# deepika090/HL-HGAT

Hardware: AMD Instinct MI355X
Metric: graphs/sec HL-HGAT fwd+bwd, ZINC-12k simplex graphs, 1/2/4/8 MI355X (higher is better)
Workload: dtype fp32; 1 GPU; BASELINE configs[1]: ZINC-12k-scale, HL_HGCNN_zinc_dense_int3_pyr channels=[2,2,2] filters=[64,64,64] K=3 mlp=[256,256] keig=15; step = copy of the device-resident batch into the step's static buffers + fwd + L1 + bwd (+ grad all-reduce) + Adam; the batch tables (Laplacian / incidence CSRs, degrees, segment offsets) are built by the data loader at collate time, outside the step (see loader); graphs_per_gpu=1000, global_batch=1000, parallelism=dp1

## Files before the change

hl-hgat_amd/csrc/bn.hip:

```cpp
#include "gemm_core.h"

#include <atomic>
#include <cstdlib>

using namespace hlhgat;

namespace {

constexpr int kThreads = 256;
constexpr int kMaxParts = 512;
constexpr int kFlatMax = 256;
constexpr int kGroup = 16;
constexpr int kMaxGroups = kMaxParts / kGroup;
constexpr int kMaxTiles = 1024;
constexpr int kGridBase = kMaxTiles * (1 + kMaxGroups);
constexpr int kCounters = kGridBase + 2 * kMaxTiles;
constexpr int kMaxSlots = 4096;
constexpr int APPLY_RPT = 2;
constexpr int kMaxRpt = 32;

struct BnLayout {
  int v;
  int tpr;
  int rp;
// ... 92 lines not shown
}

struct StatsArgs {
  const int32_t* nvalid;
  const float* x;
  int64_t ldx;
  const float* y;
  int64_t ldy;
  const float* dy;
  int64_t lddy;
  int64_t n;
  int C;
  int tpr, rp, tiles, parts;
  int64_t rows_per_part;
  double* part;
  double* gpart;
  unsigned* count;
  const float* weight;
  const float* bias;
  float* running_mean;
  float* running_var;
  int64_t* nbt;
  float momentum, eps;
  float* save_mean;
  float* save_invstd;
  float* coef;
  float* dweight;
  float* dbias;
  float* out;
  int64_t ldo;
  int relu;
  unsigned wait_us;
  unsigned* err;
  unsigned long long* slots;
  double* sums_out;
  int flat_max;
};

typedef __attribute__((address_space(1))) unsigned long long gu64_t;
__device__ __forceinline__ void st_wt(double* p, double v) {
  __hip_atomic_store((gu64_t*)p, (unsigned long long)__double_as_longlong(v), __ATOMIC_RELAXED,
                     __HIP_MEMORY_SCOPE_AGENT);
}
__device__ __forceinline__ double ld_wt(const double* p) {
  return __longlong_as_double(
      (long long)__hip_atomic_load((gu64_t*)p, __ATOMIC_RELAXED, __HIP_MEMORY_SCOPE_AGENT));
}

__device__ unsigned g_bn_wait_timeouts = 0;
__device__ unsigned g_bn_log_n = 0;
__device__ hlhgat_bn_giveup_t g_bn_log[HLHGAT_BN_LOG_MAX];

constexpr uint64_t kTicksPerUs = 100;
enum : unsigned { kKidBnGrid = 1, kKidProjBn = 2 };

__device__ __forceinline__ void report_state_error(unsigned* err) {
  if (err) __hip_atomic_store(err, (unsigned)HLHGAT_DEVERR_BN_STATE, __ATOMIC_RELAXED,
                              __HIP_MEMORY_SCOPE_SYSTEM);
}

__device__ __forceinline__ bool arrive_last(unsigned* counter, unsigned total, unsigned* err) {
  __shared__ unsigned s_last;
  asm volatile("s_waitcnt vmcnt(0)" ::: "memory");
  __syncthreads();
  if (threadIdx.x == 0) {
    unsigned prev = __hip_atomic_fetch_add(counter, 1u, __ATOMIC_RELAXED,
                                           __HIP_MEMORY_SCOPE_AGENT);
    s_last = (prev == total - 1) ? 1u : 0u;
    if (prev >= total) report_state_error(err);
    if (s_last)
      __hip_atomic_store(counter, 0u, __ATOMIC_RELAXED, __HIP_MEMORY_SCOPE_AGENT);
  }
  __syncthreads();
  return s_last != 0u;
}

typedef __attribute__((address_space(1))) unsigned long long gu64c_t;

__device__ __forceinline__ unsigned long long slot_mark(unsigned gen0) {
  return ((unsigned long long)gen0 << 2) | 1ull;
}

__device__ __forceinline__ bool poll_gen(unsigned long long* word, unsigned gen0,
                                         unsigned wait_us) {
  const uint64_t t0 = __builtin_amdgcn_s_memrealtime();
  const uint64_t lim = (uint64_t)wait_us * kTicksPerUs;
  for (;;) {
    const unsigned long long w =
        __hip_atomic_load((gu64c_t*)word, __ATOMIC_RELAXED, __HIP_MEMORY_SCOPE_AGENT);
    if ((unsigned)(w >> 32) != gen0) return true;
    if (__builtin_amdgcn_s_memrealtime() - t0 >= lim) return false;
    __builtin_amdgcn_s_sleep(2);
  }
}

__device__ __forceinline__ bool give_up(unsigned long long* word, unsigned long long* slot,
                                        unsigned gen0, unsigned kid, const unsigned* arr,
                                        bool arr_low64, unsigned total, unsigned wait_us) {
  const unsigned long long mark = slot_mark(gen0);
  __hip_atomic_store((gu64c_t*)slot, mark, __ATOMIC_SEQ_CST, __HIP_MEMORY_SCOPE_AGENT);
  const unsigned long long w =
      __hip_atomic_load((gu64c_t*)word, __ATOMIC_SEQ_CST, __HIP_MEMORY_SCOPE_AGENT);
  bool mine = false;
  if ((unsigned)(w >> 32) != gen0) {
    unsigned long long exp = mark;
    mine = __hip_atomic_compare_exchange_strong((gu64c_t*)slot, &exp, mark + 1ull,
                                                __ATOMIC_SEQ_CST, __ATOMIC_SEQ_CST,
// ... 460 lines not shown
        if (a.y) yv[u] = vload<V>(a.y + rr * a.ldy + c);
      }
#pragma unroll
      for (int u = 0; u < 4; ++u) acc(xv[u], gv[u], yv[u]);
    }
    for (; r < r_hi; r += a.rp) {
      vt xv = vload<V>(a.x + r * a.ldx + c);
      vt gv = vload<V>(a.dy + r * a.lddy + c);
      vt yv = gv;
      if (a.y) yv = vload<V>(a.y + r * a.ldy + c);
      acc(xv, gv, yv);
    }
  }
  write_partials<V, kThreads>(s0, s1, a, c0, blk);
  __shared__ double sum0[kThreads], sum1[kThreads];
  const int tile_c = a.tpr * V;
  if (!last_reduce<kThreads>(a, c0, tile_c, sum0, sum1, blk)) return;
  if (a.sums_out) {
    write_sums(a, c0, tile_c, sum0, sum1, n_eff, blk);
    for (int t = threadIdx.x; t < tile_c; t += kThreads) {
      const int cc = c0 + t;
      if (cc >= a.C) continue;
      if (a.dweight) a.dweight[cc] = (float)(sum1[t] * (double)a.save_invstd[cc]);
      if (a.dbias) a.dbias[cc] = (float)sum0[t];
    }
    return;
  }
  for (int t = threadIdx.x; t < tile_c; t += kThreads) {
    const int cc = c0 + t;
    if (cc >= a.C) continue;
    float A, B, Cc;
    bwd_coefs(a.save_invstd[cc], a.weight ? a.weight[cc] : 1.f, sum0[t], sum1[t], n_eff, A, B,
              Cc);
    if (a.dweight) a.dweight[cc] = (float)(sum1[t] * (double)a.save_invstd[cc]);
    if (a.dbias) a.dbias[cc] = (float)sum0[t];
    a.coef[cc] = A;
    a.coef[a.C + cc] = B;
    a.coef[2 * a.C + cc] = Cc;
  }
}

template <int V>
__global__ __launch_bounds__(kThreads) void k_bn_bwd_reduce(StatsArgs a) {
  k_bn_bwd_reduce_body<V>(a, blk_hw());
}

void launch_bwd_reduce(bool vec, dim3 grid, hipStream_t st, ProfScope* prof, const StatsArgs& s) {
  if (vec)
    launch(k_bn_bwd_reduce<4>, grid, dim3(kThreads), 0, st, prof, s);
  else
    launch(k_bn_bwd_reduce<1>, grid, dim3(kThreads), 0, st, prof, s);
}

template <int V>
__device__ __forceinline__ void k_bn_bwd_apply_body(const BwdApplyArgs& a, Blk blk) {
  using vt = typename VecT<V>::type;
  const int cl = threadIdx.x % a.tpr;
  const int rg = threadIdx.x / a.tpr;
  const int c = blk.y * a.tpr * V + cl * V;
  if (c >= a.C) return;
  float A[V], B[V], Cc[V], mu[V];
#pragma unroll
  for (int v = 0; v < V; ++v) {
    A[v] = a.coef[c + v];
    B[v] = a.coef[a.C + c + v];
    Cc[v] = a.coef[2 * a.C + c + v];
    mu[v] = a.mean[c + v];
  }
  const int64_t n_eff = eff_rows(a.n, a.nvalid);
  const int64_t r0 = (int64_t)blk.x * a.rp * APPLY_RPT + rg;
  vt xv[APPLY_RPT], gv[APPLY_RPT], yv[APPLY_RPT];
#pragma unroll
  for (int u = 0; u < APPLY_RPT; ++u) {
    const int64_t r = r0 + u * a.rp;
    if (r < n_eff) {
      xv[u] = vload<V>(a.x + r * a.ldx + c);
      gv[u] = vload<V>(a.dy + r * a.lddy + c);
      if (a.y) yv[u] = vload<V>(a.y + r * a.ldy + c);
    }
  }
#pragma unroll
  for (int u = 0; u < APPLY_RPT; ++u) {
    const int64_t r = r0 + u * a.rp;
    if (r >= a.n) break;
    vt o;
#pragma unroll
    for (int v = 0; v < V; ++v) {
      float g = vget(gv[u], v);
      if (a.y && !(vget(yv[u], v) > 0.f)) g = 0.f;
      vget(o, v) = r >= n_eff ? 0.f : A[v] * g + (B[v] * (vget(xv[u], v) - mu[v]) + Cc[v]);
    }
    vstore<V>(a.dx + r * a.lddx + c, o);
  }
}

template <int V>
__global__ __launch_bounds__(kThreads) void k_bn_bwd_apply(BwdApplyArgs a) {
  k_bn_bwd_apply_body<V>(a, blk_hw());
}

struct SyncArgs {
  const int32_t* nvalid;
  const float* x;
  int64_t ldx;
  const float* y;
  int64_t ldy;
  const float* dy;
  int64_t lddy;
  float* out;
  int64_t ldo;
  int64_t n;
  int C;
  int tpr, rp;
  const double* gathered;
  int world;
  const float* weight;
  const float* bias;
  float* running_mean;
  float* running_var;
  int64_t* nbt;
  float momentum, eps;
  float* save_mean;
  float* save_invstd;
  int relu;
};

__device__ __forceinline__ void sync_totals(const SyncArgs& a, int cc, double& s0, double& s1,
                                            double& cnt) {
  s0 = s1 = cnt = 0.0;
  const int64_t stride = 2 * (int64_t)a.C + 1;
  for (int r = 0; r < a.world; ++r) {
    const double* g = a.gathered + r * stride;
    s0 += g[cc];
    s1 += g[a.C + cc];
    cnt += g[2 * a.C];
  }
}

template <int V>
__global__ __launch_bounds__(kThreads) void k_bn_sync_apply(SyncArgs a) {
  using vt = typename VecT<V>::type;
  const int cl = threadIdx.x % a.tpr;
  const int rg = threadIdx.x / a.tpr;
// ... 364 lines not shown
    }
  }
  __syncthreads();
#pragma unroll
  for (int tn = 0; tn < kPbTN; ++tn) {
    const int cl = tn * 16 + i, cc = n_base + cl;
    const float sc = (s.weight ? s.weight[cc] : 1.f) * ss[cl];
    const float mu = sm[cl];
    const float sh = s.bias ? s.bias[cc] : 0.f;
#pragma unroll
    for (int r = 0; r < 4; ++r) {
      const float z = (acc[tn][r] - mu) * sc + sh;
      acc[tn][r] = m_base + 4 * q + r >= n_eff ? 0.f : ((s.relu && z < 0.f) ? 0.f : z);
    }
  }
  const bool vy = (s.ldo % 4) == 0 && (reinterpret_cast<uintptr_t>(s.out) & 15) == 0;
  store_tile_rows<kPbTN>(acc, scratch, m_base, g.M, s.out + n_base, s.ldo, kPbTN * 16, nullptr,
                         0, vy);
  pb_stamp<STAMPS>(a, 5, pb_now());
  if (!top) return;
  __shared__ unsigned char taken[kMaxParts];
  if (!take_left<kThreads>(tile_slots, parts, s_gen0, taken)) return;
  __builtin_amdgcn_fence(__ATOMIC_ACQUIRE, "agent");
  const int c4 = threadIdx.x & 15, rr = threadIdx.x >> 4;
  float sc[4], mu[4], sh[4];
#pragma unroll
  for (int v = 0; v < 4; ++v) {
    const int cl = 4 * c4 + v, cc = n_base + cl;
    sc[v] = (s.weight ? s.weight[cc] : 1.f) * ss[cl];
    mu[v] = sm[cl];
    sh[v] = s.bias ? s.bias[cc] : 0.f;
  }
  for (int p = 0; p < parts; ++p) {
    if (!taken[p]) continue;
    for (int64_t r = (int64_t)p * 64 + rr; r < (int64_t)p * 64 + 64 && r < g.M; r += 16) {
      float4 xv;
      const float* xp = g.C + r * g.ldc + n_base + 4 * c4;
      if (vx) xv = *reinterpret_cast<const float4*>(xp);
      else xv = make_float4(xp[0], xp[1], xp[2], xp[3]);
      const float4 o = bn_row_out<4>(xv, mu, sc, sh, r >= n_eff, s.relu);
      float* yp = s.out + r * s.ldo + n_base + 4 * c4;
      if (vy) {
        *reinterpret_cast<float4*>(yp) = o;
      } else {
        yp[0] = o.x;
        yp[1] = o.y;
        yp[2] = o.z;
        yp[3] = o.w;
      }
    }
  }
}

bool& proj_bn_fused_flag() {
  static bool v = true;
  return v;
}

bool& proj_bn_split_flag() {
  static bool v = false;
  return v;
}

bool bn_vec_ok(int64_t C, std::initializer_list<int64_t> lds,
               std::initializer_list<const void*> ptrs) {
  if (C % 4) return false;
  for (int64_t ld : lds)
    if (ld % 4) return false;
  for (const void* p : ptrs)
    if (p && !aligned16(p)) return false;
  return true;
}

unsigned apply_grid_x(int64_t n, int rp) {
  int64_t g = ceil_div(n, (int64_t)rp * APPLY_RPT);
  if (g < 1) g = 1;
  return (unsigned)g;
}

StatsArgs stats_args(const BnLayout& L, const BnWs& w, const float* x, int64_t ldx, int64_t n,
                     const int32_t* n_valid, int64_t C) {
  StatsArgs s{};
  s.nvalid = n_valid;
  s.x = x;
  s.ldx = ldx;
  s.n = n;
  s.C = (int)C;
  s.tpr = L.tpr;
  s.rp = L.rp;
  s.tiles = L.tiles;
  s.parts = L.parts;
  s.rows_per_part = L.rows_per_part;
  s.part = w.part;
  s.gpart = w.gpart;
  s.count = w.count;
  s.slots = w.slots;
  s.err = hlhgat::device_error_word();
  s.flat_max = kFlatMax;
  return s;
}

unsigned g_wait_us = 1000;

int64_t capacity_of(const void* kernel) {
  static auto* cache = new std::vector<std::pair<const void*, int64_t>>();
  for (const auto& kv : *cache)
    if (kv.first == kernel) return kv.second;
  int dev = 0, cus = 0, occ = 0;
  int64_t c = 0;
  static const int share = [] {
    const char* e = std::getenv("HLHGAT_BN_COLOCATE");
    const int v = e ? std::atoi(e) : 2;
    return v >= 1 && v <= 16 ? v : 2;
  }();
  if (hipGetDevice(&dev) == hipSuccess &&
      hipDeviceGetAttribute(&cus, hipDeviceAttributeMultiprocessorCount, dev) == hipSuccess &&
      hipOccupancyMaxActiveBlocksPerMultiprocessor(&occ, kernel, kThreads, 0) == hipSuccess)
    c = (int64_t)occ * cus / share;
  cache->push_back({kernel, c});
  return c;
}

int rpt_bucket(const BnLayout& L) {
  const int64_t need = ceil_div(L.rows_per_part, (int64_t)L.rp);
  if (need > kMaxRpt) return 0;
  for (int r : {2, 4, 8, 16, 32})
    if (need <= r) return r;
  return 0;
}


using GridFn = void (*)(StatsArgs);

GridFn fwd_grid_fn(bool vec, int rpt) {
  switch (rpt * 2 + (vec ? 1 : 0)) {
    case 4: return k_bn_fwd_grid<1, 2>;
    case 5: return k_bn_fwd_grid<4, 2>;
    case 8: return k_bn_fwd_grid<1, 4>;
    case 9: return k_bn_fwd_grid<4, 4>;
    case 16: return k_bn_fwd_grid<1, 8>;
    case 17: return k_bn_fwd_grid<4, 8>;
    case 32: return k_bn_fwd_grid<1, 16>;
    case 33: return k_bn_fwd_grid<4, 16>;
    case 64: return k_bn_fwd_grid<1, 32>;
    case 65: return k_bn_fwd_grid<4, 32>;
    default: return nullptr;
  }
}

GridFn pick_grid(const BnLayout& L, bool vec) {
  if (!bn_one_launch() || L.parts > kFlatMax) return nullptr;
  const int64_t grid = (int64_t)L.parts * L.tiles;
  const int rpt = rpt_bucket(L);
  GridFn f = rpt ? fwd_grid_fn(vec, rpt) : nullptr;
  const int64_t cap = f ? capacity_of(reinterpret_cast<const void*>(f)) : 0;
  if (!f || grid > 256 || grid > cap) return nullptr;
  return f;
}


}


extern "C" int64_t hlhgat_bn_workspace_bytes(int64_t n, int64_t C) {
  if (n < 0 || C <= 0) return 0;
  return (int64_t)bn_ws_bytes(n, C);
}

extern "C" int hlhgat_bn_stats_train(const float* x, int64_t ldx, int64_t n,
                                     const int32_t* n_valid, int64_t C, float* running_mean,
                                     float* running_var, int64_t* num_batches_tracked,
                                     float momentum, float eps, float* save_mean,
                                     float* save_invstd, void* workspace,
                                     int64_t workspace_bytes, void* stream) {
  HLH_CHECK_ARG(n >= 1 && C >= 1 && C < (1 << 20) && ldx >= C,
                "bn_stats_train: bad sizes n=%lld C=%lld", (long long)n, (long long)C);
  HLH_CHECK_ARG(x && save_mean && save_invstd, "bn_stats_train: NULL pointer");
  HLH_CHECK_ARG((running_mean == nullptr) == (running_var == nullptr),
                "bn_stats_train: running_mean/var must both be given or both NULL");
  HLH_CHECK_ARG(workspace && workspace_bytes >= (int64_t)bn_ws_bytes(n, C),
                "bn_stats_train: workspace too small");
  const bool vec = bn_vec_ok(C, {ldx}, {x});
  BnLayout L = bn_layout(n, C, vec);
  HLH_CHECK_ARG(L.tiles <= kMaxTiles, "bn_stats_train: C too large");
  StatsArgs s = stats_args(L, carve(workspace, n, C), x, ldx, n, n_valid, C);
  s.running_mean = running_mean;
  s.running_var = running_var;
  s.nbt = num_batches_tracked;
  s.momentum = momentum;
  s.eps = eps;
  s.save_mean = save_mean;
  s.save_invstd = save_invstd;
  hipStream_t st = as_stream(stream);
  dim3 g1(L.parts, L.tiles);
  if (vec)
    launch(k_bn_stats<4>, dim3(g1), dim3(kThreads), 0, st, nullptr, s);
  else
    launch(k_bn_stats<1>, dim3(g1), dim3(kThreads), 0, st, nullptr, s);
  HLH_CHECK_LAUNCH();
  return HLHGAT_OK;
}

extern "C" int hlhgat_bn_apply(const float* x, int64_t ldx, int64_t n, const int32_t* n_valid,
                               int64_t C, const float* weight, const float* bias,
                               const float* save_mean, const float* save_invstd, int relu,
                               float* y, int64_t ldy, void* stream) {
  HLH_CHECK_ARG(n >= 1 && C >= 1 && C < (1 << 20) && ldx >= C && ldy >= C,
                "bn_apply: bad sizes n=%lld C=%lld", (long long)n, (long long)C);
  HLH_CHECK_ARG(x && y && save_mean && save_invstd, "bn_apply: NULL pointer");
  const bool vec = bn_vec_ok(C, {ldx, ldy}, {x, y});
  BnLayout L = bn_layout(n, C, vec);
  HLH_CHECK_ARG(L.tiles <= kMaxTiles, "bn_apply: C too large");
// ... 211 lines not shown
      launch(k_bn_apply<1>, g2, dim3(kThreads), 0, st, nullptr, p);
    HLH_CHECK_LAUNCH();
  }
  return HLHGAT_OK;
}

extern "C" int hlhgat_set_proj_bn_split(int on) {
  proj_bn_split_flag() = on != 0;
  return HLHGAT_OK;
}

extern "C" int hlhgat_set_proj_bn_fused(int on) {
  proj_bn_fused_flag() = on != 0;
  return HLHGAT_OK;
}

extern "C" int hlhgat_proj_bn_fused_capacity(int64_t* out) {
  HLH_CHECK_ARG(out, "proj_bn_fused_capacity: NULL pointer");
  *out = capacity_of(reinterpret_cast<const void*>(k_proj_bn_fwd<false>));
  return HLHGAT_OK;
}

extern "C" int hlhgat_bn_bwd_train(const float* x, int64_t ldx, const float* y,
                                   int64_t ldy, const float* dy, int64_t lddy,
                                   int64_t n, const int32_t* n_valid, int64_t C,
                                   const float* weight,
                                   const float* save_mean, const float* save_invstd,
                                   float* dx, int64_t lddx, float* dweight,
                                   float* dbias, void* workspace,
                                   int64_t workspace_bytes, void* stream) {
  HLH_CHECK_ARG(n >= 1 && C >= 1 && ldx >= C && lddy >= C && lddx >= C && (!y || ldy >= C),
                "bn_bwd_train: bad sizes");
  HLH_CHECK_ARG(x && dy && dx && save_mean && save_invstd, "bn_bwd_train: NULL pointer");
  HLH_CHECK_ARG(workspace && workspace_bytes >= (int64_t)bn_ws_bytes(n, C),
                "bn_bwd_train: workspace too small");
  const bool vec = bn_vec_ok(C, {ldx, lddy, lddx, y ? ldy : 4}, {x, y, dy, dx});
  BnLayout L = bn_layout(n, C, vec, bn_bwd_min_parts());
  HLH_CHECK_ARG(L.tiles <= kMaxTiles, "bn_bwd_train: C too large");
  BnWs w = carve(workspace, n, C);
  StatsArgs s = stats_args(L, w, x, ldx, n, n_valid, C);
  s.flat_max = bn_bwd_flat_max();
  s.y = y;
  s.ldy = ldy;
  s.dy = dy;
  s.lddy = lddy;
  s.weight = weight;
  s.save_mean = const_cast<float*>(save_mean);
  s.save_invstd = const_cast<float*>(save_invstd);
  s.coef = w.coef;
  s.dweight = dweight;
  s.dbias = dbias;
  hipStream_t st = as_stream(stream);
  dim3 g1(L.parts, L.tiles);
  {
    ProfScope prof(HLHGAT_PROF_BN_BWD, st, (y ? 12.0 : 8.0) * (double)n * C, 0.0);
    if (vec)
      launch_bwd_reduce(true, g1, st, &prof, s);
    else
      launch_bwd_reduce(false, g1, st, &prof, s);
  }
  HLH_CHECK_LAUNCH();
  BwdApplyArgs p{n_valid, x, ldx, y, ldy, dy, lddy, dx, lddx, n, (int)C, w.coef, save_mean,
                 L.tpr, L.rp};
  dim3 g2(apply_grid_x(n, L.rp), L.tiles);
  if (vec)
    launch(k_bn_bwd_apply<4>, dim3(g2), dim3(kThreads), 0, st, nullptr, p);
  else
    launch(k_bn_bwd_apply<1>, dim3(g2), dim3(kThreads), 0, st, nullptr, p);
  HLH_CHECK_LAUNCH();
  return HLHGAT_OK;
}

extern "C" int hlhgat_bn_bwd_reduce(const float* x, int64_t ldx, const float* y, int64_t ldy,
                                    const float* dy, int64_t lddy, int64_t n,
                                    const int32_t* n_valid, int64_t C, const float* weight,
                                    const float* save_mean, const float* save_invstd,
                                    float* coef, float* dweight, float* dbias, void* workspace,
                                    int64_t workspace_bytes, void* stream) {
  HLH_CHECK_ARG(n >= 1 && C >= 1 && ldx >= C && lddy >= C && (!y || ldy >= C),
                "bn_bwd_reduce: bad sizes");
  HLH_CHECK_ARG(x && dy && coef && save_mean && save_invstd, "bn_bwd_reduce: NULL pointer");
  HLH_CHECK_ARG(workspace && workspace_bytes >= (int64_t)bn_ws_bytes(n, C),
                "bn_bwd_reduce: workspace too small");
  const bool vec = bn_vec_ok(C, {ldx, lddy, y ? ldy : 4}, {x, y, dy});
  BnLayout L = bn_layout(n, C, vec, bn_bwd_min_parts());
  HLH_CHECK_ARG(L.tiles <= kMaxTiles, "bn_bwd_reduce: C too large");
  BnWs w = carve(workspace, n, C);
  StatsArgs s = stats_args(L, w, x, ldx, n, n_valid, C);
  s.flat_max = bn_bwd_flat_max();
  s.y = y;
  s.ldy = ldy;
  s.dy = dy;
  s.lddy = lddy;
  s.weight = weight;
  s.save_mean = const_cast<float*>(save_mean);
  s.save_invstd = const_cast<float*>(save_invstd);
  s.coef = coef;
  s.dweight = dweight;
  s.dbias = dbias;
  hipStream_t st = as_stream(stream);
  ProfScope prof(HLHGAT_PROF_BN_BWD, st, (y ? 12.0 : 8.0) * (double)n * C, 0.0);
  if (vec)
    launch_bwd_reduce(true, dim3(L.parts, L.tiles), st, &prof, s);
  else
    launch_bwd_reduce(false, dim3(L.parts, L.tiles), st, &prof, s);
  HLH_CHECK_LAUNCH();
// ... 105 lines not shown
    launch_bwd_reduce(false, dim3(g1), as_stream(stream), nullptr, s);
  HLH_CHECK_LAUNCH();
  return HLHGAT_OK;
}

extern "C" int hlhgat_bn_sync_bwd_apply(const float* x, int64_t ldx, const float* y,
                                        int64_t ldy, const float* dy, int64_t lddy, int64_t n,
                                        const int32_t* n_valid, int64_t C, const float* weight,
                                        const float* save_mean, const float* save_invstd,
                                        const double* gathered, int world, float* dx,
                                        int64_t lddx, void* stream) {
  HLH_CHECK_ARG(n >= 1 && C >= 1 && ldx >= C && lddy >= C && lddx >= C && (!y || ldy >= C) &&
                    world >= 1,
                "bn_sync_bwd_apply: bad sizes");
  HLH_CHECK_ARG(x && dy && dx && gathered && save_mean && save_invstd,
                "bn_sync_bwd_apply: NULL pointer");
  const bool vec = bn_vec_ok(C, {ldx, lddy, lddx, y ? ldy : 4}, {x, y, dy, dx});
  const BnLayout L = bn_layout(n, C, vec);
  SyncArgs a{};
  a.nvalid = n_valid;
  a.x = x;
  a.ldx = ldx;
  a.y = y;
  a.ldy = ldy;
  a.dy = dy;
  a.lddy = lddy;
  a.out = dx;
  a.ldo = lddx;
  a.n = n;
  a.C = (int)C;
  a.tpr = L.tpr;
  a.rp = L.rp;
  a.gathered = gathered;
  a.world = world;
  a.weight = weight;
  a.save_mean = const_cast<float*>(save_mean);
  a.save_invstd = const_cast<float*>(save_invstd);
  dim3 g2(apply_grid_x(n, L.rp), L.tiles);
  if (vec)
    launch(k_bn_sync_bwd_apply<4>, dim3(g2), dim3(kThreads), 0, as_stream(stream), nullptr, a);
  else
    launch(k_bn_sync_bwd_apply<1>, dim3(g2), dim3(kThreads), 0, as_stream(stream), nullptr, a);
  HLH_CHECK_LAUNCH();
  return HLHGAT_OK;
}

extern "C" int hlhgat_set_bn_one_launch(int on) {
  bn_one_launch_flag() = on != 0;
  return HLHGAT_OK;
}

extern "C" int hlhgat_get_bn_one_launch(void) { return bn_one_launch_flag() ? 1 : 0; }

extern "C" int hlhgat_set_bn_wait_us(unsigned wait_us) {
  g_wait_us = wait_us;
  return HLHGAT_OK;
}

extern "C" int hlhgat_bn_wait_timeouts(unsigned* out) {
  HLH_CHECK_ARG(out, "bn_wait_timeouts: NULL pointer");
  HLH_CHECK_HIP(hipMemcpyFromSymbol(out, HIP_SYMBOL(g_bn_wait_timeouts), sizeof(unsigned)));
  return HLHGAT_OK;
}

extern "C" int hlhgat_bn_giveup_log(hlhgat_bn_giveup_t* out, int max, int* logged) {
  HLH_CHECK_ARG(logged && (max <= 0 || out), "bn_giveup_log: NULL pointer");
  unsigned n = 0;
  HLH_CHECK_HIP(hipMemcpyFromSymbol(&n, HIP_SYMBOL(g_bn_log_n), sizeof(unsigned)));
  *logged = (int)n;
  int k = (int)n < HLHGAT_BN_LOG_MAX ? (int)n : HLHGAT_BN_LOG_MAX;
  if (k > max) k = max;
  if (k > 0)
    HLH_CHECK_HIP(hipMemcpyFromSymbol(out, HIP_SYMBOL(g_bn_log), sizeof(hlhgat_bn_giveup_t) * k));
  return HLHGAT_OK;
}

extern "C" int hlhgat_bn_giveup_reset(void) {
  const unsigned z = 0;
  HLH_CHECK_HIP(hipDeviceSynchronize());
  HLH_CHECK_HIP(hipMemcpyToSymbol(HIP_SYMBOL(g_bn_log_n), &z, sizeof(unsigned)));
  HLH_CHECK_HIP(hipMemcpyToSymbol(HIP_SYMBOL(g_bn_wait_timeouts), &z, sizeof(unsigned)));
  return HLHGAT_OK;
}
```

hl-hgat_amd/csrc/runtime.hip:

```cpp
#include "common.h"

#include <cstring>
#include <mutex>
#include <vector>

namespace hlhgat {

static thread_local std::string g_last_error;

void set_error(const char* fmt, ...) {
  char buf[1024];
  va_list ap;
  va_start(ap, fmt);
  vsnprintf(buf, sizeof(buf), fmt, ap);
  va_end(ap);
  g_last_error = buf;
}

namespace {
constexpr int kPoolSize = 1 << 14;
struct ProfClass {
  bool enabled = false;
  std::vector<hipEvent_t> start, stop;
  std::vector<double> bytes, flops;
  int used = 0;
  int64_t dropped = 0;
};
std::mutex g_prof_mu;
ProfClass g_prof[HLHGAT_PROF_NCLASS];
}

ProfScope::ProfScope(int kernel_class, hipStream_t s, double b, double f)
    : cls(kernel_class), bytes(b), flops(f) {
  (void)s;
  if (kernel_class < 0 || kernel_class >= HLHGAT_PROF_NCLASS) return;
  std::lock_guard<std::mutex> lk(g_prof_mu);
  ProfClass& pc = g_prof[kernel_class];
  if (!pc.enabled) return;
  if (pc.used >= (int)pc.start.size()) {
    pc.dropped++;
    return;
  }
  slot = pc.used++;
  pc.bytes[slot] = b;
  pc.flops[slot] = f;
  start_ev = pc.start[slot];
  stop_ev = pc.stop[slot];
}

namespace {
std::mutex g_err_mu;
unsigned* g_err_word = nullptr;
}

unsigned* device_error_word() {
  std::lock_guard<std::mutex> lk(g_err_mu);
  if (!g_err_word) {
    void* p = nullptr;
    hipError_t e = hipHostMalloc(&p, 64, hipHostMallocPortable | hipHostMallocMapped |
                                             hipHostMallocCoherent);
    if (e != hipSuccess) {
      set_error("hipHostMalloc(device error word) failed: %s", hipGetErrorString(e));
      return nullptr;
    }
    *static_cast<volatile unsigned*>(p) = 0u;
    g_err_word = static_cast<unsigned*>(p);
  }
  return g_err_word;
}

}

using namespace hlhgat;

extern "C" int hlhgat_version(void) { return 103; }

extern "C" int hlhgat_device_errors(unsigned* out) {
  HLH_CHECK_ARG(out, "device_errors: NULL pointer");
  unsigned* w = device_error_word();
  HLH_CHECK_ARG(w, "device_errors: %s", hlhgat_last_error());
  *out = *static_cast<volatile unsigned*>(w);
  return HLHGAT_OK;
}

extern "C" int hlhgat_clear_device_errors(void) {
  unsigned* w = device_error_word();
  HLH_CHECK_ARG(w, "clear_device_errors: %s", hlhgat_last_error());
  *static_cast<volatile unsigned*>(w) = 0u;
  return HLHGAT_OK;
}

extern "C" const char* hlhgat_last_error(void) { return g_last_error.c_str(); }

extern "C" int hlhgat_stream_create(int device, unsigned flags, int priority,
                                    const uint32_t* cu_mask, int cu_mask_words, void** out) {
  HLH_CHECK_ARG(out && device >= 0 && cu_mask_words >= 0 && (cu_mask_words == 0 || cu_mask) &&
                    (cu_mask_words == 0 || priority == 0),
                "stream_create: bad arguments (a CU-masked stream has the default priority)");
  int prev = 0;
  HLH_CHECK_HIP(hipGetDevice(&prev));
  HLH_CHECK_HIP(hipSetDevice(device));
  hipStream_t s = nullptr;
  hipError_t e;
  if (cu_mask_words > 0) {
    int cus = 0;
    e = hipDeviceGetAttribute(&cus, hipDeviceAttributeMultiprocessorCount, device);
    int on = 0;
    for (int w = 0; w < cu_mask_words; ++w) on += __builtin_popcount(cu_mask[w]);
    if (e == hipSuccess && (on == 0 || cu_mask_words * 32 < cus)) {
      (void)hipSetDevice(prev);
      HLH_CHECK_ARG(false, "stream_create: the CU mask must cover all %d CUs (%d words given) "
                    "and enable at least one", cus, cu_mask_words);
    }
    if (e == hipSuccess) e = hipExtStreamCreateWithCUMask(&s, (uint32_t)cu_mask_words, cu_mask);
  } else if (priority != 0) {
    e = hipStreamCreateWithPriority(&s, flags, priority);
  } else {
    e = hipStreamCreateWithFlags(&s, flags);
  }
  (void)hipSetDevice(prev);
  HLH_CHECK_HIP(e);
  *out = s;
  return HLHGAT_OK;
}

extern "C" int hlhgat_stream_cu_mask(void* stream, uint32_t* cu_mask, int cu_mask_words) {
  HLH_CHECK_ARG(stream && cu_mask && cu_mask_words > 0, "stream_cu_mask: bad arguments");
  HLH_CHECK_HIP(hipExtStreamGetCUMask(as_stream(stream), (uint32_t)cu_mask_words, cu_mask));
// ... 385 lines not shown
```

hl-hgat_amd/hlhgat/_lib.py:

```python
from __future__ import annotations

import ctypes as C
import os

import torch

_HERE = os.path.dirname(os.path.abspath(__file__))
LIB_PATH = os.environ.get("HLHGAT_LIB", os.path.join(_HERE, "libhlhgat.so"))

c_i32, c_i64, c_f32, c_f64, c_vp, c_sz = (C.c_int32, C.c_int64, C.c_float,
                                           C.c_double, C.c_void_p, C.c_size_t)
P_i64 = C.POINTER(c_i64)
P_i32 = C.POINTER(c_i32)
P_f64 = C.POINTER(c_f64)
P_vp = C.POINTER(c_vp)

MAX_COPY_BLOCKS = 64

SIGNATURES = {
    "hlhgat_version": (c_i32, []),
    "hlhgat_last_error": (C.c_char_p, []),
    "hlhgat_csr_workspace_bytes": (c_sz, [c_i64]),
    "hlhgat_csr_from_coo": (c_i32, [c_vp, c_vp, c_vp, c_i64, c_i64, c_i64, c_vp, c_vp,
                                    c_vp, c_vp, c_vp, c_sz, c_vp]),
# ... 14 lines not shown
                            c_vp, c_i64, c_vp]),
    "hlhgat_poly_step": (c_i32, [c_vp, c_vp, c_vp, c_vp, c_i64, c_i64, c_vp, c_vp, c_vp,
                                 c_i64, c_i64, c_vp, c_i64, c_vp, c_i64, c_vp, c_i64, c_f32,
                                 c_f32, c_f32, c_f32, c_f32, c_f32, c_vp, c_i64, c_vp]),
    "hlhgat_incidence_step": (c_i32, [c_vp, c_vp, c_vp, c_vp, c_i64, c_i64, c_i64, c_vp, c_i64,
                                      c_i64, c_vp, c_i64, c_f32, c_f32, c_vp, c_i64, c_vp]),
    "hlhgat_poly_basis_fwd": (c_i32, [c_i32, c_vp, c_vp, c_vp, c_i64, c_i64, c_vp, c_vp,
                                      c_vp, c_i64, c_i64, c_i32, c_vp, c_vp]),
    "hlhgat_poly_basis_bwd": (c_i32, [c_i32, c_vp, c_vp, c_vp, c_i64, c_i64, c_vp, c_vp,
                                      c_i64, c_i32, c_vp, c_vp]),
    "hlhgat_hodge_factor_work_floats": (c_i64, [c_i64, c_i64]),
    "hlhgat_hodge_spmm": (c_i32, [c_vp, c_vp, c_i64, c_i64, c_vp, c_i64, c_vp, c_vp]),
    "hlhgat_hodge_poly_step": (c_i32, [c_vp, c_vp, c_i64, c_i64, c_vp, c_i64, c_vp, c_i64, c_vp,
                                       c_i64, c_f32, c_f32, c_f32, c_f32, c_f32, c_f32, c_vp,
                                       c_i64, c_vp, c_vp]),
    "hlhgat_poly_basis_fwd_factored": (c_i32, [c_i32, c_vp, c_vp, c_i64, c_i64, c_i32, c_vp,
                                               c_vp, c_vp]),
    "hlhgat_poly_basis_bwd_factored": (c_i32, [c_i32, c_vp, c_i64, c_i32, c_vp, c_vp, c_vp]),
    "hlhgat_hodge_lmax_workspace_bytes": (c_i64, [c_i64, c_i32]),
    "hlhgat_hodge_lmax": (c_i32, [c_vp, c_vp, c_vp, c_i64, c_i64, c_vp, c_i64, c_i32, c_vp, c_vp,
                                  c_i64, c_vp]),
    "hlhgat_bn_bwd_reduce": (c_i32, [c_vp, c_i64, c_vp, c_i64, c_vp, c_i64, c_i64, c_vp, c_i64,
                                     c_vp, c_vp, c_vp, c_vp, c_vp, c_vp, c_vp, c_i64, c_vp]),
    "hlhgat_eig_pe_workspace_bytes": (c_i64, [c_i64, c_i64, c_i32]),
    "hlhgat_eig_pe": (c_i32, [c_vp, c_vp, c_vp, c_i64, c_i64, c_vp, c_i64, c_i64, c_i32, c_vp,
                              c_i64, c_vp, c_vp, c_i64, c_vp]),
    "hlhgat_hodge_row_sizes": (c_i32, [c_vp, c_vp, c_i64, c_i64, c_vp, c_vp, c_vp]),
    "hlhgat_hodge_build": (c_i32, [c_vp, c_vp, c_vp, c_i64, c_i64, c_vp, c_vp, c_vp, c_vp, c_i64,
                                   c_vp, c_vp, c_vp, c_i64, c_vp]),
    "hlhgat_proj_fwd": (c_i32, [c_i32, P_vp, P_i64, P_vp, P_i64, P_i64, c_i64, c_i64, c_vp,
                                c_vp, c_i64, c_i32, c_vp]),
    "hlhgat_proj_bwd_data": (c_i32, [c_i32, c_vp, c_i64, P_vp, P_i64, P_i64, c_i64, c_i64,
                                     P_vp, P_i64, c_i32, c_vp]),
    "hlhgat_proj_bwd_weight_workspace_floats": (c_i64, [c_i32, P_i64, c_i64, c_i64, c_i32]),
    "hlhgat_proj_bwd_weight": (c_i32, [c_i32, c_vp, c_i64, P_vp, P_i64, P_i64, c_i64, c_i64,
                                       P_vp, P_i64, c_vp, c_i32, c_vp, c_i64, c_vp]),
    "hlhgat_proj_bwd": (c_i32, [c_i64, c_i64, c_vp, c_i64, c_i32, P_vp, P_i64, P_i64, P_vp,
                                P_i64, c_vp, c_i32, P_vp, P_i64, P_i64, P_vp, P_i64, c_i32,
                                c_vp, c_i64, c_vp]),
    "hlhgat_proj_bwd_defer": (c_i32, [c_i64, c_i64, c_vp, c_i64, c_i32, P_vp, P_i64, P_i64,
                                      P_vp, P_i64, c_vp, c_i32, P_vp, P_i64, P_i64, P_vp, P_i64,
                                      c_i32, c_vp, c_i64, c_vp, c_vp, c_vp, c_vp]),
    "hlhgat_reduce_run": (c_i32, [c_vp, c_vp]),
    "hlhgat_proj_bn_fwd": (c_i32, [c_i32, P_vp, P_i64, P_vp, P_i64, P_i64, c_i64, c_i64, c_vp,
                                   c_vp, c_i64, c_vp, c_vp, c_vp, c_vp, c_vp, c_vp, c_f32,
                                   c_f32, c_i32, c_vp, c_i64, c_vp, c_vp, c_vp, c_i64, c_vp]),
    "hlhgat_set_proj_bn_fused": (c_i32, [c_i32]),
    "hlhgat_set_proj_bn_split": (c_i32, [c_i32]),
    "hlhgat_set_proj_bwd_rows": (c_i32, [c_i32]),
    "hlhgat_set_gemm_big": (c_i32, [c_i32, c_i64]),
    "hlhgat_proj_bn_fused_capacity": (c_i32, [P_i64]),
    "hlhgat_set_bn_one_launch": (c_i32, [c_i32]),
    "hlhgat_get_bn_one_launch": (c_i32, []),
    "hlhgat_set_bn_wait_us": (c_i32, [C.c_uint32]),
    "hlhgat_set_proj_bn_stamps": (c_i32, [c_vp, c_i64]),
    "hlhgat_bn_giveup_log": (c_i32, [c_vp, c_i32, c_vp]),
    "hlhgat_bn_giveup_reset": (c_i32, []),
    "hlhgat_test_occupy": (c_i32, [c_i32, c_i32, c_i32, C.c_uint32, c_vp]),
    "hlhgat_device_errors": (c_i32, [c_vp]),
    "hlhgat_stream_create": (c_i32, [c_i32, C.c_uint32, c_i32, c_vp, c_i32, c_vp]),
    "hlhgat_stream_cu_mask": (c_i32, [c_vp, c_vp, c_i32]),
    "hlhgat_clear_device_errors": (c_i32, []),
    "hlhgat_bn_wait_timeouts": (c_i32, [c_vp]),
    "hlhgat_edge_gather2": (c_i32, [c_vp, c_i64, c_vp, c_i64, c_i64, c_vp, c_vp, c_f32,
                                    c_f32, c_vp, c_i64, c_vp, c_i64, c_i32, c_vp]),
    "hlhgat_att_score_fwd": (c_i32, [c_i64, c_i64, c_vp, c_i64, c_vp, c_i64, c_vp, c_i64,
                                     c_f32, c_f32, c_f32, c_i32, c_vp, c_vp]),
    "hlhgat_att_score_bwd": (c_i32, [c_i64, c_i64, c_vp, c_i64, c_vp, c_i64, c_vp, c_i64,
                                     c_f32, c_f32, c_f32, c_i32, c_vp, c_vp, c_vp, c_vp,
                                     c_vp, c_i64, c_vp]),
    "hlhgat_segment_mean_fwd": (c_i32, [c_vp, c_vp, c_i64, c_vp, c_i64, c_i64, c_vp, c_i64,
                                        c_vp]),
    "hlhgat_segment_mean_bwd": (c_i32, [c_vp, c_vp, c_i64, c_vp, c_i64, c_i64, c_vp, c_i64,
                                        c_i64, c_vp]),
    "hlhgat_row_scale_fwd": (c_i32, [c_i64, c_i64, c_vp, c_i64, c_vp, c_vp, c_i64, c_vp]),
    "hlhgat_row_scale_bwd": (c_i32, [c_i64, c_i64, c_vp, c_i64, c_vp, c_vp, c_i64, c_vp, c_i64,
                                     c_vp, c_vp]),
    "hlhgat_dropout_fwd": (c_i32, [c_vp, c_i64, c_i64, c_i64, C.c_uint32, c_f32, c_vp,
                                   C.c_uint32, c_vp, c_vp, c_i64, c_vp]),
    "hlhgat_dropout_bwd": (c_i32, [c_vp, c_i64, c_i64, c_i64, C.c_uint32, c_f32, c_vp,
                                   C.c_uint32, c_vp, c_i64, c_vp]),
    "hlhgat_dropout_advance": (c_i32, [c_vp, c_vp]),
    "hlhgat_edge_absdiff": (c_i32, [c_vp, c_i64, c_vp, c_i64, c_i64, c_vp, c_i64, c_vp, c_i64,
                                    c_vp]),
    "hlhgat_pool_mean_bwd": (c_i32, [c_vp, c_vp, c_i64, c_vp, c_i64, c_i64, c_vp, c_i64,
                                     c_i64, c_vp]),
    "hlhgat_bn_workspace_bytes": (c_i64, [c_i64, c_i64]),
    "hlhgat_bn_apply_running": (c_i32, [c_vp, c_i64, c_i64, c_i64, c_vp, c_vp, c_vp, c_vp, c_f32,
                                        c_i32, c_vp, c_i64, c_vp]),
    "hlhgat_bn_fwd_train": (c_i32, [c_vp, c_i64, c_i64, c_vp, c_i64, c_vp, c_vp, c_vp, c_vp,
                                    c_vp, c_f32, c_f32, c_i32, c_vp, c_i64, c_vp, c_vp, c_vp,
                                    c_i64, c_vp]),
    "hlhgat_bn_bwd_train": (c_i32, [c_vp, c_i64, c_vp, c_i64, c_vp, c_i64, c_i64, c_vp, c_i64,
                                    c_vp, c_vp, c_vp, c_vp, c_i64, c_vp, c_vp, c_vp, c_i64,
                                    c_vp]),
    "hlhgat_adam_prepare": (c_i32, [c_vp, c_i64, c_vp, c_vp]),
    "hlhgat_adam_flat_prepared": (c_i32, [c_vp, c_vp, c_vp, c_vp, c_i64, c_vp, c_f64, c_f64,
                                          c_f64, c_f64, c_f64, c_vp]),
    "hlhgat_adam_flat": (c_i32, [c_vp, c_vp, c_vp, c_vp, c_i64, c_vp, c_f64, c_f64, c_f64,
                                 c_f64, c_f64, c_vp]),
    "hlhgat_bce_logits_fwd": (c_i32, [c_vp, c_vp, c_i64, c_f32, c_vp, c_vp]),
    "hlhgat_bce_logits_bwd": (c_i32, [c_vp, c_vp, c_i64, c_f32, c_vp, c_vp, c_vp]),
    "hlhgat_l1_loss_fwd": (c_i32, [c_vp, c_vp, c_i64, c_vp, c_vp]),
    "hlhgat_l1_loss_bwd": (c_i32, [c_vp, c_vp, c_i64, c_vp, c_vp, c_vp]),
    "hlhgat_loss_workspace_bytes": (c_sz, [c_i64]),
    "hlhgat_bce_reduce_fwd": (c_i32, [c_vp, c_vp, c_vp, c_i64, c_i32, c_i32, c_f32, c_f32, c_f32,
# ... 124 lines not shown
```

include/hlhgat.h:

```cpp
#ifndef HLHGAT_H_
#define HLHGAT_H_

#include <stddef.h>
#include <stdint.h>

#ifdef __cplusplus
extern "C" {
#endif

#define HLHGAT_OK 0
#define HLHGAT_EINVAL 1
#define HLHGAT_EHIP 2

#define HLHGAT_POLY_LAGUERRE 0
#define HLHGAT_POLY_CHEB 1
#define HLHGAT_POLY_LAGUERRE_DEMO 2

#define HLHGAT_SIGMA_SIGMOID 0
#define HLHGAT_SIGMA_RELU 1

int hlhgat_version(void);
const char* hlhgat_last_error(void);

size_t hlhgat_csr_workspace_bytes(int64_t nnz);
// ... 255 lines not shown
                         int64_t lddx, float* da, void* stream);

int hlhgat_segment_mean_fwd(const int32_t* seg_ptr, const int32_t* seg_rows,
                            int64_t n_seg, const float* x, int64_t ldx,
                            int64_t d, float* out, int64_t ldo, void* stream);
int hlhgat_segment_mean_bwd(const int32_t* seg_ptr, const int32_t* seg_rows,
                            int64_t n_seg, const float* dout, int64_t ldo,
                            int64_t d, float* dx, int64_t ldx, int64_t n_rows,
                            void* stream);

int hlhgat_pool_mean_bwd(const int32_t* seg_ptr, const int32_t* seg_rows,
                         int64_t n_seg, const float* dout, int64_t ldo,
                         int64_t d, float* dx, int64_t ldx, int64_t n_rows,
                         void* stream);

int64_t hlhgat_bn_workspace_bytes(int64_t n, int64_t C);
int hlhgat_bn_apply_running(const float* x, int64_t ldx, int64_t n, int64_t C,
                            const float* weight, const float* bias, const float* running_mean,
                            const float* running_var, float eps, int relu, float* y,
                            int64_t ldy, void* stream);
int hlhgat_bn_fwd_train(const float* x, int64_t ldx, int64_t n,
                        const int32_t* n_valid, int64_t C,
                        const float* weight, const float* bias,
                        float* running_mean, float* running_var,
                        int64_t* num_batches_tracked, float momentum, float eps,
                        int relu, float* y, int64_t ldy, float* save_mean,
                        float* save_invstd, void* workspace,
                        int64_t workspace_bytes, void* stream);
int hlhgat_bn_stats_train(const float* x, int64_t ldx, int64_t n, const int32_t* n_valid,
                          int64_t C, float* running_mean, float* running_var,
                          int64_t* num_batches_tracked, float momentum, float eps,
                          float* save_mean, float* save_invstd, void* workspace,
                          int64_t workspace_bytes, void* stream);
int hlhgat_bn_apply(const float* x, int64_t ldx, int64_t n, const int32_t* n_valid, int64_t C,
                    const float* weight, const float* bias, const float* save_mean,
                    const float* save_invstd, int relu, float* y, int64_t ldy, void* stream);

int hlhgat_proj_bn_fwd(int nblocks, const float* const* A, const int64_t* lda,
                       const float* const* W, const int64_t* ldw, const int64_t* kb, int64_t M,
                       int64_t N, const float* bias, float* x, int64_t ldx,
                       const int32_t* n_valid, const float* bn_weight, const float* bn_bias,
                       float* running_mean, float* running_var, int64_t* num_batches_tracked,
                       float momentum, float eps, int relu, float* y, int64_t ldy,
                       float* save_mean, float* save_invstd, void* workspace,
                       int64_t workspace_bytes, void* stream);
int hlhgat_set_gemm_big(int mode, int64_t min_m);
int hlhgat_set_proj_bwd_rows(int on);
int hlhgat_set_proj_bn_fused(int on);
int hlhgat_set_proj_bn_split(int on);
int hlhgat_set_proj_bn_stamps(void* buf, int64_t words);
int hlhgat_proj_bn_fused_capacity(int64_t* out);
int hlhgat_set_bn_one_launch(int on);
int hlhgat_get_bn_one_launch(void);
int hlhgat_set_bn_wait_us(unsigned wait_us);

int hlhgat_bn_wait_timeouts(unsigned* out);
#define HLHGAT_BN_LOG_MAX 64
typedef struct {
  uint32_t kernel;
  uint32_t tile;
  uint32_t block;
  uint32_t total;
  uint32_t arrivals;
  uint32_t gen0;
  uint32_t gen_seen;
  uint32_t wait_us;
  uint32_t outcome;
} hlhgat_bn_giveup_t;
int hlhgat_bn_giveup_log(hlhgat_bn_giveup_t* out, int max, int* logged);
int hlhgat_bn_giveup_reset(void);

int hlhgat_bn_bwd_reduce(const float* x, int64_t ldx, const float* y, int64_t ldy,
                         const float* dy, int64_t lddy, int64_t n, const int32_t* n_valid,
                         int64_t C, const float* weight, const float* save_mean,
                         const float* save_invstd, float* coef, float* dweight, float* dbias,
                         void* workspace, int64_t workspace_bytes, void* stream);
int hlhgat_bn_bwd_train(const float* x, int64_t ldx, const float* y, int64_t ldy,
                        const float* dy, int64_t lddy, int64_t n,
                        const int32_t* n_valid, int64_t C,
                        const float* weight, const float* save_mean,
                        const float* save_invstd, float* dx, int64_t lddx,
                        float* dweight, float* dbias, void* workspace,
                        int64_t workspace_bytes, void* stream);

int64_t hlhgat_bn_sums_len(int64_t C);
int hlhgat_bn_sums_fwd(const float* x, int64_t ldx, const float* y, int64_t ldy, int64_t n,
                       const int32_t* n_valid, int64_t C, double* sums, void* workspace,
                       int64_t workspace_bytes, void* stream);
int hlhgat_bn_sync_fwd_apply(const float* x, int64_t ldx, int64_t n, const int32_t* n_valid,
                             int64_t C, const double* gathered, int world, const float* weight,
                             const float* bias, float* running_mean, float* running_var,
                             int64_t* num_batches_tracked, float momentum, float eps, int relu,
                             float* y, int64_t ldy, float* save_mean, float* save_invstd,
                             void* stream);
int hlhgat_bn_sums_bwd(const float* x, int64_t ldx, const float* y, int64_t ldy,
                       const float* dy, int64_t lddy, float* dx_layout, int64_t lddx, int64_t n,
                       const int32_t* n_valid, int64_t C, const float* save_mean,
                       const float* save_invstd, double* sums, float* dweight, float* dbias,
                       void* workspace, int64_t workspace_bytes, void* stream);
int hlhgat_bn_sync_bwd_apply(const float* x, int64_t ldx, const float* y, int64_t ldy,
                             const float* dy, int64_t lddy, int64_t n, const int32_t* n_valid,
                             int64_t C, const float* weight, const float* save_mean,
                             const float* save_invstd, const double* gathered, int world,
                             float* dx, int64_t lddx, void* stream);

int hlhgat_adam_flat(float* param, const float* grad, float* exp_avg, float* exp_avg_sq,
// ... 127 lines not shown
```

Baseline: 369,300 graphs/s.

## Fuse BN backward reduce and apply into one grid-synchronized launch

Adds a single-launch BatchNorm backward kernel. Each block holds its rows' masked gradients and centered inputs in registers, reduces per-channel sums through partials, and the last arriving block computes coefficients and publishes a generation flag. The other blocks spin-wait on that flag and then apply dx from their registers, which removes the second launch and the re-read of x, dy and y. In exchange it relies on inter-block polling, which is only safe when all blocks are co-resident, so it is gated by a grid-size and occupancy capacity check and keeps a give-up path that handles the rows of blocks that never arrived.

```diff
diff --git a/hl-hgat_amd/csrc/bn.hip b/hl-hgat_amd/csrc/bn.hip
--- a/hl-hgat_amd/csrc/bn.hip
+++ b/hl-hgat_amd/csrc/bn.hip
@@ -168,7 +168,7 @@
 __device__ hlhgat_bn_giveup_t g_bn_log[HLHGAT_BN_LOG_MAX];
 
 constexpr uint64_t kTicksPerUs = 100;
-enum : unsigned { kKidBnGrid = 1, kKidProjBn = 2 };
+enum : unsigned { kKidBnGrid = 1, kKidProjBn = 2, kKidBnBwd = 3 };
 
 __device__ __forceinline__ void report_state_error(unsigned* err) {
   if (err) __hip_atomic_store(err, (unsigned)HLHGAT_DEVERR_BN_STATE, __ATOMIC_RELAXED,
@@ -735,6 +735,10 @@
     launch(k_bn_bwd_reduce<1>, grid, dim3(kThreads), 0, st, prof, s);
 }
 
+__device__ __forceinline__ float bn_dx(float A, float g, float B, float xc, float Cc) {
+  return A * g + (B * xc + Cc);
+}
+
 template <int V>
 __device__ __forceinline__ void k_bn_bwd_apply_body(const BwdApplyArgs& a, Blk blk) {
   using vt = typename VecT<V>::type;
@@ -771,7 +775,7 @@
     for (int v = 0; v < V; ++v) {
       float g = vget(gv[u], v);
       if (a.y && !(vget(yv[u], v) > 0.f)) g = 0.f;
-      vget(o, v) = r >= n_eff ? 0.f : A[v] * g + (B[v] * (vget(xv[u], v) - mu[v]) + Cc[v]);
+      vget(o, v) = r >= n_eff ? 0.f : bn_dx(A[v], g, B[v], vget(xv[u], v) - mu[v], Cc[v]);
     }
     vstore<V>(a.dx + r * a.lddx + c, o);
   }
@@ -1242,7 +1246,198 @@
   }
 }
 
+template <int V, int RPT>
+__device__ __forceinline__ void k_bn_bwd_grid_body(const StatsArgs& a, Blk blk) {
+  using vt = typename VecT<V>::type;
+  constexpr int CH = RPT < 4 ? RPT : 4;
+  __shared__ unsigned s_gen0, s_ok;
+  const int cl = threadIdx.x % a.tpr;
+  const int rg = threadIdx.x / a.tpr;
+  const int c0 = blk.y * a.tpr * V;
+  const int c = c0 + cl * V;
+  const int64_t r_lo = (int64_t)blk.x * a.rows_per_part;
+  const int64_t n_eff = eff_rows(a.n, a.nvalid);
+  int64_t r_hi = r_lo + a.rows_per_part;
+  if (r_hi > n_eff) r_hi = n_eff;
+  vt gr[RPT], xcr[RPT];
+  double s0[V], s1[V];
+  float mu[V];
+#pragma unroll
+  for (int v = 0; v < V; ++v) {
+    s0[v] = s1[v] = 0.0;
+    mu[v] = (c + v < a.C) ? a.save_mean[c + v] : 0.f;
+  }
+#pragma unroll
+  for (int j = 0; j < RPT; ++j)
+#pragma unroll
+    for (int v = 0; v < V; ++v) vget(gr[j], v) = vget(xcr[j], v) = 0.f;
+  const bool has_y = a.y != nullptr;
+  const float* mp = has_y ? a.y : a.dy;
+  const int64_t ldm = has_y ? a.ldy : a.lddy;
+  if (c < a.C) {
+#pragma unroll
+    for (int j0 = 0; j0 < RPT; j0 += CH) {
+      vt xv[CH], gv[CH], yv[CH];
+#pragma unroll
+      for (int u = 0; u < CH; ++u) {
+        const int64_t r = r_lo + rg + (int64_t)(j0 + u) * a.rp;
+        const int64_t rr = r < r_hi ? r : 0;
+        xv[u] = vload<V>(a.x + rr * a.ldx + c);
+        gv[u] = vload<V>(a.dy + rr * a.lddy + c);
+        yv[u] = vload<V>(mp + rr * ldm + c);
+      }
+#pragma unroll
+      for (int u = 0; u < CH; ++u) {
+        const int64_t r = r_lo + rg + (int64_t)(j0 + u) * a.rp;
+        if (r < r_hi) {
+#pragma unroll
+          for (int v = 0; v < V; ++v) {
+            float g = vget(gv[u], v);
+            if (has_y && !(vget(yv[u], v) > 0.f)) g = 0.f;
+            const float xc = vget(xv[u], v) - mu[v];
+            vget(gr[j0 + u], v) = g;
+            vget(xcr[j0 + u], v) = xc;
+            s0[v] += (double)g;
+            s1[v] += (double)g * (double)xc;
+          }
+        }
+      }
+    }
+  }
+  const int tile_c = a.tpr * V;
+  const int fc = c0 + (int)threadIdx.x;
+  const bool fcol = (int)threadIdx.x < tile_c && fc < a.C;
+  const float f_is = fcol ? a.save_invstd[fc] : 0.f;
+  const float f_w = (fcol && a.weight) ? a.weight[fc] : 1.f;
+  write_partials<V, kThreads>(s0, s1, a, c0, blk);
+  unsigned long long* word = gen_word(a, blk.y);
+  if (threadIdx.x == 0)
+    s_gen0 = (unsigned)(__hip_atomic_load((gu64c_t*)word, __ATOMIC_RELAXED,
+                                          __HIP_MEMORY_SCOPE_AGENT) >> 32);
+  __shared__ double sum0[kThreads], sum1[kThreads];
+  __shared__ float sA[kThreads], sB[kThreads], sC[kThreads];
+  unsigned long long* tile_slots = a.slots + (int64_t)blk.y * blk.gx;
+  const bool fin = last_reduce<kThreads>(a, c0, tile_c, sum0, sum1, blk);
+  if (fin) {
+    if ((int)threadIdx.x < tile_c) {
+      const int t = threadIdx.x, cc = fc;
+      float A = 0.f, B = 0.f, Cc = 0.f;
+      if (fcol) {
+        bwd_coefs(f_is, f_w, sum0[t], sum1[t], n_eff, A, B, Cc);
+        if (a.dweight) a.dweight[cc] = (float)(sum1[t] * (double)f_is);
+        if (a.dbias) a.dbias[cc] = (float)sum0[t];
+        __hip_atomic_store(reinterpret_cast<unsigned*>(a.coef + cc), __float_as_uint(A),
+                           __ATOMIC_RELAXED, __HIP_MEMORY_SCOPE_AGENT);
+        __hip_atomic_store(reinterpret_cast<unsigned*>(a.coef + a.C + cc), __float_as_uint(B),
+                           __ATOMIC_RELAXED, __HIP_MEMORY_SCOPE_AGENT);
+        __hip_atomic_store(reinterpret_cast<unsigned*>(a.coef + 2 * a.C + cc),
+                           __float_as_uint(Cc), __ATOMIC_RELAXED, __HIP_MEMORY_SCOPE_AGENT);
+      }
+      sA[t] = A;
+      sB[t] = B;
+      sC[t] = Cc;
+    }
+    asm volatile("s_waitcnt vmcnt(0)" ::: "memory");
+    __syncthreads();
+    if (threadIdx.x == 0) publish_gen(word, 1ull << 32);
+  } else {
+    if (threadIdx.x == 0) {
+      unsigned ok = poll_gen(word, s_gen0, a.wait_us) ? 1u : 0u;
+      if (!ok) {
+        const unsigned total = a.parts <= a.flat_max
+                                   ? (unsigned)a.parts
+                                   : (unsigned)((a.parts + kGroup - 1) / kGroup);
+        ok = give_up(word, tile_slots + blk.x, s_gen0, kKidBnBwd, a.count + blk.y, false, total,
+                     a.wait_us)
+                 ? 1u
+                 : 0u;
+      }
+      s_ok = ok;
+    }
+    __syncthreads();
+    if (!s_ok) return;
+    for (int t = threadIdx.x; t < tile_c; t += kThreads) {
+      const int cc = c0 + t;
+      float A = 0.f, B = 0.f, Cc = 0.f;
+      if (cc < a.C) {
+        A = __uint_as_float(__hip_atomic_load(reinterpret_cast<unsigned*>(a.coef + cc),
+                                              __ATOMIC_RELAXED, __HIP_MEMORY_SCOPE_AGENT));
+        B = __uint_as_float(__hip_atomic_load(reinterpret_cast<unsigned*>(a.coef + a.C + cc),
+                                              __ATOMIC_RELAXED, __HIP_MEMORY_SCOPE_AGENT));
+        Cc = __uint_as_float(__hip_atomic_load(reinterpret_cast<unsigned*>(a.coef + 2 * a.C + cc),
+                                               __ATOMIC_RELAXED, __HIP_MEMORY_SCOPE_AGENT));
+      }
+      sA[t] = A;
+      sB[t] = B;
+      sC[t] = Cc;
+    }
+  }
+  __syncthreads();
+  float A[V], B[V], Cc[V];
+#pragma unroll
+  for (int v = 0; v < V; ++v) {
+    A[v] = sA[cl * V + v];
+    B[v] = sB[cl * V + v];
+    Cc[v] = sC[cl * V + v];
+  }
+  if (c < a.C) {
+    int64_t r_end = r_lo + a.rows_per_part;
+    if (r_end > a.n) r_end = a.n;
+#pragma unroll
+    for (int j = 0; j < RPT; ++j) {
+      const int64_t r = r_lo + rg + (int64_t)j * a.rp;
+      if (r < r_end) {
+        vt o;
+#pragma unroll
+        for (int v = 0; v < V; ++v)
+          vget(o, v) =
+              r >= n_eff ? 0.f : bn_dx(A[v], vget(gr[j], v), B[v], vget(xcr[j], v), Cc[v]);
+        vstore<V>(a.out + r * a.ldo + c, o);
+      }
+    }
+  }
+  if (!fin) return;
+  __shared__ unsigned char taken[kMaxParts];
+  if (!take_left<kThreads>(tile_slots, (int)blk.gx, s_gen0, taken)) return;
+  if (c >= a.C) return;
+  for (unsigned p = 0; p < blk.gx; ++p) {
+    if (!taken[p]) continue;
+    const int64_t p_lo = (int64_t)p * a.rows_per_part;
+    int64_t p_end = p_lo + a.rows_per_part;
+    if (p_end > a.n) p_end = a.n;
+    for (int64_t r = p_lo + rg; r < p_end; r += a.rp) {
+      vt o;
+      if (r < n_eff) {
+        vt xv = vload<V>(a.x + r * a.ldx + c);
+        vt gv = vload<V>(a.dy + r * a.lddy + c);
+        vt yv = gv;
+        if (a.y) yv = vload<V>(a.y + r * a.ldy + c);
+#pragma unroll
+        for (int v = 0; v < V; ++v) {
+          float g = vget(gv, v);
+          if (a.y && !(vget(yv, v) > 0.f)) g = 0.f;
+          vget(o, v) = bn_dx(A[v], g, B[v], vget(xv, v) - mu[v], Cc[v]);
+        }
+      } else {
+#pragma unroll
+        for (int v = 0; v < V; ++v) vget(o, v) = 0.f;
+      }
+      vstore<V>(a.out + r * a.ldo + c, o);
+    }
+  }
+}
+
+template <int V, int RPT>
+__global__ __launch_bounds__(kThreads) void k_bn_bwd_grid(StatsArgs a) {
+  k_bn_bwd_grid_body<V, RPT>(a, blk_hw());
+}
+
 bool& proj_bn_fused_flag() {
+  static bool v = true;
+  return v;
+}
+
+bool& bn_bwd_one_launch_flag() {
   static bool v = true;
   return v;
 }
@@ -1348,6 +1543,31 @@
   return f;
 }
 
+GridFn bwd_grid_fn(bool vec, int rpt) {
+  switch (rpt * 2 + (vec ? 1 : 0)) {
+    case 4: return k_bn_bwd_grid<1, 2>;
+    case 5: return k_bn_bwd_grid<4, 2>;
+    case 8: return k_bn_bwd_grid<1, 4>;
+    case 9: return k_bn_bwd_grid<4, 4>;
+    case 16: return k_bn_bwd_grid<1, 8>;
+    case 17: return k_bn_bwd_grid<4, 8>;
+    case 32: return k_bn_bwd_grid<1, 16>;
+    case 33: return k_bn_bwd_grid<4, 16>;
+    case 64: return k_bn_bwd_grid<1, 32>;
+    case 65: return k_bn_bwd_grid<4, 32>;
+    default: return nullptr;
+  }
+}
+
+GridFn pick_bwd_grid(const BnLayout& L, bool vec) {
+  if (!bn_one_launch() || !bn_bwd_one_launch_flag()) return nullptr;
+  const int64_t grid = (int64_t)L.parts * L.tiles;
+  const int rpt = rpt_bucket(L);
+  GridFn f = rpt ? bwd_grid_fn(vec, rpt) : nullptr;
+  const int64_t cap = f ? capacity_of(reinterpret_cast<const void*>(f)) : 0;
+  if (!f || grid > 256 || grid > cap) return nullptr;
+  return f;
+}
 
 }
 
@@ -1665,6 +1885,16 @@
   s.dbias = dbias;
   hipStream_t st = as_stream(stream);
   dim3 g1(L.parts, L.tiles);
+  if (GridFn f = pick_bwd_grid(L, vec)) {
+    s.out = dx;
+    s.ldo = lddx;
+    s.wait_us = g_wait_us;
+    HLH_CHECK_ARG(s.err, "bn_bwd_train: no device error word (%s)", hlhgat_last_error());
+    ProfScope prof(HLHGAT_PROF_BN_BWD, st, (y ? 16.0 : 12.0) * (double)n * C, 0.0);
+    launch(f, g1, dim3(kThreads), 0, st, &prof, s);
+    HLH_CHECK_LAUNCH();
+    return HLHGAT_OK;
+  }
   {
     ProfScope prof(HLHGAT_PROF_BN_BWD, st, (y ? 12.0 : 8.0) * (double)n * C, 0.0);
     if (vec)
@@ -1876,6 +2106,13 @@
 
 extern "C" int hlhgat_get_bn_one_launch(void) { return bn_one_launch_flag() ? 1 : 0; }
 
+extern "C" int hlhgat_set_bn_bwd_one_launch(int on) {
+  bn_bwd_one_launch_flag() = on != 0;
+  return HLHGAT_OK;
+}
+
+extern "C" int hlhgat_get_bn_bwd_one_launch(void) { return bn_bwd_one_launch_flag() ? 1 : 0; }
+
 extern "C" int hlhgat_set_bn_wait_us(unsigned wait_us) {
   g_wait_us = wait_us;
   return HLHGAT_OK;
diff --git a/hl-hgat_amd/csrc/runtime.hip b/hl-hgat_amd/csrc/runtime.hip
--- a/hl-hgat_amd/csrc/runtime.hip
+++ b/hl-hgat_amd/csrc/runtime.hip
@@ -73,7 +73,7 @@
 
 using namespace hlhgat;
 
-extern "C" int hlhgat_version(void) { return 103; }
+extern "C" int hlhgat_version(void) { return 104; }
 
 extern "C" int hlhgat_device_errors(unsigned* out) {
   HLH_CHECK_ARG(out, "device_errors: NULL pointer");
diff --git a/hl-hgat_amd/hlhgat/_lib.py b/hl-hgat_amd/hlhgat/_lib.py
--- a/hl-hgat_amd/hlhgat/_lib.py
+++ b/hl-hgat_amd/hlhgat/_lib.py
@@ -90,6 +90,8 @@
     "hlhgat_proj_bn_fused_capacity": (c_i32, [P_i64]),
     "hlhgat_set_bn_one_launch": (c_i32, [c_i32]),
     "hlhgat_get_bn_one_launch": (c_i32, []),
+    "hlhgat_set_bn_bwd_one_launch": (c_i32, [c_i32]),
+    "hlhgat_get_bn_bwd_one_launch": (c_i32, []),
     "hlhgat_set_bn_wait_us": (c_i32, [C.c_uint32]),
     "hlhgat_set_proj_bn_stamps": (c_i32, [c_vp, c_i64]),
     "hlhgat_bn_giveup_log": (c_i32, [c_vp, c_i32, c_vp]),
diff --git a/include/hlhgat.h b/include/hlhgat.h
--- a/include/hlhgat.h
+++ b/include/hlhgat.h
@@ -331,6 +331,8 @@
 int hlhgat_proj_bn_fused_capacity(int64_t* out);
 int hlhgat_set_bn_one_launch(int on);
 int hlhgat_get_bn_one_launch(void);
+int hlhgat_set_bn_bwd_one_launch(int on);
+int hlhgat_get_bn_bwd_one_launch(void);
 int hlhgat_set_bn_wait_us(unsigned wait_us);
 
 int hlhgat_bn_wait_timeouts(unsigned* out);
```

Result: faster. 382,000 graphs/s (median of 6 runs) (+3.4%).
